# bartelvdh/Navtex

Measured on AMD Instinct MI355X. Metric: IQ Msamples/s through FIR->FSK->bitsync, higher is better.
Workload: dtype f64

## Files before the change

### navtex_amd/csrc/nvx_demod.hip

```cpp
#include <hip/hip_runtime.h>
#include <stdint.h>
#include <stdlib.h>

#include "nvx_tables.h"
#include "nvx_atan2.h"
#include "nvx_fsm.h"
#include "nvx_kernels.h"

enum { DS_Y3 = 0, DS_DPHI = 8, DS_S = 16, DS_C = 24, DS_COUNT = 24 + 567 };
enum { DI_SYNCED = 0, DI_SYNC_OFF, DI_NEXT_SYNC_OFF, DI_PHASE, DI_PREV_OFFSET, DI_COUNT };
static_assert(DI_COUNT == NVX_DEMOD_INTS && DS_COUNT == NVX_DEMOD_DOUBLES && DI_PREV_OFFSET == NVX_DI_PREV_OFFSET &&
              DI_PHASE == NVX_DI_PHASE, "state layout");

#ifndef NVX_FRONT_THREADS
#define NVX_FRONT_THREADS 128
#endif
#ifndef DTL
#define DTL NVX_FRONT_TILE
static_assert(DTL % 9 == 0, "a tile is a whole number of bit periods");
#endif
#define FRONT_SLIDE ((567 + NVX_FRONT_THREADS - 1) / NVX_FRONT_THREADS)
#define G_DAB 8
#define G_CB 574
#define G_CSA 582

__device__ __forceinline__ double2 y3_at(const double2 *y3, const double *hist, int t)
{
    if (t >= 0) return y3[t];
    double2 r; r.x = hist[2 * (4 + t)]; r.y = hist[2 * (4 + t) + 1];
    return r;
}

__device__ __forceinline__ double front_dphi(double2 s, double2 p)
{
    const double prodReal = s.x * p.x + s.y * p.y;
    const double prodImg  = s.y * p.x - s.x * p.y;
    return nvx_atan2(prodImg, prodReal);
}
__device__ __forceinline__ void front_energies(double2 w0, double2 w1, double2 w2, double2 w3, double2 w4,
                                               float &Brot, float &Yrot)
{
    float BR = 0.0f, BI = 0.0f, YR = 0.0f, YI = 0.0f;
#pragma unroll
    for (int i = 0; i < 5; i++) {
        const double2 w = i == 0 ? w0 : i == 1 ? w1 : i == 2 ? w2 : i == 3 ? w3 : w4;
        const float fR = NVX_BF_R[i], fI = NVX_BF_I[i];
        const double sampleR = w.x, sampleI = w.y;
        YR = (float)((double)YR + ((double)((float)sampleR * fR) - sampleI * (double)fI));
        YI = (float)((double)YI + ((double)((float)sampleR * fI) + sampleI * (double)fR));
        BR = (float)((double)BR + ((double)((float)sampleR * fR) + sampleI * (double)fI));
        BI = (float)((double)BI + ((double)((float)(-sampleR) * fI) + sampleI * (double)fR));
    }
    Brot = BR * BR + BI * BI;
    Yrot = YR * YR + YI * YI;
}
__device__ __forceinline__ unsigned char front_decision(double2 w0, double2 w1, double2 w2, double2 w3, double2 w4, float &hi, float &lo)
{
    float Brot, Yrot;
    front_energies(w0, w1, w2, w3, w4, Brot, Yrot);
    const bool b = Brot > Yrot;
    hi = b ? Brot : Yrot; lo = b ? Yrot : Brot;
    return b ? 1 : 0;
}

struct FrontSig { double power, dphi_b, dphi2_b, dphi_y, dphi2_y, hi, lo; unsigned nb, pad; };
__device__ __forceinline__ void front_sig_init(FrontSig &s)
{
    s.power = s.dphi_b = s.dphi2_b = s.dphi_y = s.dphi2_y = s.hi = s.lo = 0.0; s.nb = s.pad = 0;
}
__device__ __forceinline__ void front_sig_add(FrontSig &s, double2 y, double ds, unsigned char d, float hi, float lo)
{
    s.power += y.x * y.x + y.y * y.y;
    const double b = d ? ds : 0.0, m = d ? 0.0 : ds;
    s.dphi_b += b; s.dphi2_b += b * b; s.dphi_y += m; s.dphi2_y += m * m;
    s.hi += (double)hi; s.lo += (double)lo; s.nb += d;
}
__device__ __forceinline__ double front_wave_sum(double v)
{
#pragma unroll
    for (int o = 32; o >= 1; o >>= 1) v += __shfl_xor(v, o);
    return v;
}
__device__ __forceinline__ unsigned front_wave_sum(unsigned v)
{
#pragma unroll
    for (int o = 32; o >= 1; o >>= 1) v += __shfl_xor(v, o);
    return v;
}
__device__ __forceinline__ void front_sig_publish(FrontSig s, unsigned n, FrontSig *s_w, nvx_sig_rec *rec, int tid)
{
    s.power = front_wave_sum(s.power); s.dphi_b = front_wave_sum(s.dphi_b); s.dphi2_b = front_wave_sum(s.dphi2_b);
    s.dphi_y = front_wave_sum(s.dphi_y); s.dphi2_y = front_wave_sum(s.dphi2_y); s.hi = front_wave_sum(s.hi); s.lo = front_wave_sum(s.lo);
    s.nb = front_wave_sum(s.nb);
    if ((tid & 63) == 0) s_w[tid >> 6] = s;
    __syncthreads();
    if (tid == 0) {
        FrontSig t = s_w[0];
#pragma unroll
        for (int w = 1; w < NVX_FRONT_THREADS / 64; w++) {
            const FrontSig &u = s_w[w];
            t.power += u.power; t.dphi_b += u.dphi_b; t.dphi2_b += u.dphi2_b; t.dphi_y += u.dphi_y; t.dphi2_y += u.dphi2_y;
            t.hi += u.hi; t.lo += u.lo; t.nb += u.nb;
        }
        nvx_sig_rec r;
        r.sum_power = t.power; r.sum_dphi_b = t.dphi_b; r.sum_dphi2_b = t.dphi2_b; r.sum_dphi_y = t.dphi_y; r.sum_dphi2_y = t.dphi2_y;
        r.sum_mf_hi = t.hi; r.sum_mf_lo = t.lo; r.samples = n; r.b_samples = t.nb;
        *rec = r;
    }
}
__device__ __forceinline__ double front_corr(const double *dp)
{
    double temp = 0.0;
#pragma unroll
    for (int i = 0; i < 9; i++) temp += (double)NVX_CORR_MASK[i] * dp[i];
    return __builtin_fabs(temp);
}
__device__ __forceinline__ double front_class_sum(const double *cnow, unsigned u)
{
    const unsigned c = u % 9u;
    const int d0 = (int)((u + 566u - c) % 567u);
    const int jw = d0 / 9;
    const double *run1 = cnow - d0;
    const double *run2 = run1 - 567;
    double temp = 0.0;
#pragma unroll
    for (int j = 0; j < 63; j++) temp += (j <= jw ? run1 : run2)[9 * j];
    return temp;
}
struct FrontTies { unsigned near, evals; float minm; };
__device__ __forceinline__ FrontTies front_ties_init() { FrontTies t; t.near = 0; t.evals = 0; t.minm = __uint_as_float(0x7f800000u); return t; }
__device__ __forceinline__ unsigned short front_word(const unsigned char *d9, const double *sv, bool evaluate, FrontTies &ties)
{
    unsigned w = 0;
#pragma unroll
    for (int k = 0; k < 9; k++) w |= (unsigned)d9[k] << k;
    unsigned max_index = 15;
    if (evaluate) {
        double temp_max = -1.0, runner_up = -1.0;
        max_index = 0;
#pragma unroll
        for (int i = 0; i < 9; i++) {
            const double v = sv[i];
            if (v > temp_max) { runner_up = temp_max; temp_max = v; max_index = i; }
            else if (v > runner_up) runner_up = v;
        }
        if (temp_max > 0.0) {
            const double margin = temp_max - runner_up;
            ties.evals++;
            if (margin < temp_max * 0x1p-40) ties.near++;
            ties.minm = fminf(ties.minm, (float)(margin / temp_max));
        }
    }
    return (unsigned short)(w | (max_index << 12));
}

struct FrontChain { int slot; unsigned long long g0; const double *st_rd; double *st_wr; int n3; };
__device__ __forceinline__ FrontChain front_chain(const nvx_demod_args &a, int chain_index)
{
    FrontChain c;
    c.slot = chain_index; c.g0 = a.g0; c.n3 = a.n3;
    int parity = 0;
    if (a.part) {
        const int per = 2 * a.per_part, e = chain_index / per;
        c.slot = a.part[e].stream * per + (chain_index - e * per);
        c.g0 = a.part[e].g0; parity = a.part[e].parity; c.n3 = a.part[e].n3;
    }
    c.st_rd = (parity ? a.dstate[1] : a.dstate[0]) + (size_t)c.slot * NVX_DEMOD_DOUBLES;
    c.st_wr = (parity ? a.dstate[0] : a.dstate[1]) + (size_t)c.slot * NVX_DEMOD_DOUBLES;
    return c;
}

__device__ __forceinline__ void front_publish_ties(const nvx_demod_args &a, const FrontTies &t, unsigned *s_near, unsigned *s_evals, unsigned *s_minm, int tid)
{
    if (t.evals) { atomicAdd(s_near, t.near); atomicAdd(s_evals, t.evals); atomicMin(s_minm, __float_as_uint(t.minm)); }
    __syncthreads();
    if (tid == 0 && *s_evals) {
        if (*s_near) atomicAdd(&a.ties->near_ties, (unsigned long long)*s_near);
        atomicAdd(&a.ties->evaluations, (unsigned long long)*s_evals);
        atomicMin(&a.ties->min_margin_bits, *s_minm);
    }
}

struct FrontWalkLds {
    double dphi[8 + DTL];
    double S[8 + DTL];
    double C[567 + DTL];
    unsigned char D[DTL];
    unsigned near, evals, minm;
    FrontSig sig[NVX_FRONT_THREADS / 64];
};
template <bool SIG>
__device__ __forceinline__ void front_sequential(const nvx_demod_args &a, int chain_index, int n_tiles_here, FrontWalkLds &lds)
{
    double *const s_dphi = lds.dphi, *const s_S = lds.S, *const s_C = lds.C;
    unsigned char *const s_D = lds.D;
    unsigned &s_near = lds.near, &s_evals = lds.evals, &s_minm = lds.minm;
    const int tid = threadIdx.x;
    const FrontChain ch = front_chain(a, chain_index);
    const int slot = ch.slot;
    if (!a.slot_active[slot]) return;
    if (tid == 0) { s_near = 0; s_evals = 0; s_minm = 0x7f800000u; }
    FrontTies ties = front_ties_init();
    constexpr bool sig_on = SIG;
    FrontSig sig;
    front_sig_init(sig);

    const double *st = ch.st_rd;
    const double2 *y3 = a.y3 + (size_t)slot * a.y3_cap + a.y3_base;
    double *dphi_out = a.dphi ? a.dphi + (size_t)slot * a.y3_cap + a.y3_base : nullptr;
    double *corr_out = a.corr ? a.corr + (size_t)slot * a.y3_cap + a.y3_base : nullptr;
    double *csum_out = a.csum ? a.csum + (size_t)slot * a.y3_cap + a.y3_base : nullptr;
    const double *hist = st + DS_Y3;
    if (tid < 8) { s_dphi[tid] = st[DS_DPHI + tid]; s_S[tid] = st[DS_S + tid]; }
    for (int i = tid; i < 567; i += NVX_FRONT_THREADS) s_C[i] = st[DS_C + i];
    __syncthreads();

    const int n3 = ch.n3;
    const int n_here = n_tiles_here > 0 ? min(n3, n_tiles_here * DTL) : n3;
    for (int ta = 0; ta < n_here; ta += DTL) {
        const int tl = min(DTL, n_here - ta);
        const int tl9 = (tl + 8) / 9;
        const unsigned long long gt = ch.g0 + (unsigned long long)ta;
        for (int L = tid; L < tl; L += NVX_FRONT_THREADS) {
            const int t = ta + L;
            const double2 w3 = y3_at(y3, hist, t - 1), w4 = y3[t];
            const double ds = front_dphi(w4, w3);
            s_dphi[8 + L] = ds;
            if (dphi_out) dphi_out[t] = ds;
            float hi, lo;
            const unsigned char d = front_decision(y3_at(y3, hist, t - 4), y3_at(y3, hist, t - 3), y3_at(y3, hist, t - 2), w3, w4, hi, lo);
            s_D[L] = d;
            if (sig_on && gt + L >= G_DAB) front_sig_add(sig, w4, ds, d, hi, lo);
        }
        if (tid < 9 * tl9 - tl) s_D[tl + tid] = 0;
        __syncthreads();
        for (int L = tid; L < tl; L += NVX_FRONT_THREADS)
            s_C[567 + L] = (gt + L >= G_DAB) ? front_corr(&s_dphi[L]) : 0.0;
        __syncthreads();
        const unsigned t_cb = (unsigned)((gt % 5103u + (5103u - G_CB % 5103u)) % 5103u);
        for (int L = tid; L < tl; L += NVX_FRONT_THREADS)
            s_S[8 + L] = (gt + L >= G_CB) ? front_class_sum(&s_C[567 + L], t_cb + (unsigned)L) : 0.0;
        __syncthreads();
        if (corr_out)
            for (int L = tid; L < tl; L += NVX_FRONT_THREADS) { corr_out[ta + L] = s_C[567 + L]; csum_out[ta + L] = s_S[8 + L]; }
        for (int M = tid; M < tl9; M += NVX_FRONT_THREADS) {
            const int L = 9 * M + (G_CSA % 9);
            a.words[(size_t)slot * (a.y3_cap / 9) + (ta / 9 + M)] = front_word(&s_D[9 * M], &s_S[L], L < tl && gt + L >= G_CSA, ties);
        }
        __syncthreads();
        double h_d = 0.0, h_s = 0.0, h_c[FRONT_SLIDE];
        if (tid < 8) { h_d = s_dphi[tl + tid]; h_s = s_S[tl + tid]; }
#pragma unroll
        for (int k = 0; k < FRONT_SLIDE; k++) { const int i = tid + NVX_FRONT_THREADS * k; h_c[k] = (i < 567) ? s_C[tl + i] : 0.0; }
        __syncthreads();
        if (tid < 8) { s_dphi[tid] = h_d; s_S[tid] = h_s; }
#pragma unroll
        for (int k = 0; k < FRONT_SLIDE; k++) { const int i = tid + NVX_FRONT_THREADS * k; if (i < 567) s_C[i] = h_c[k]; }
        __syncthreads();
    }

    front_publish_ties(a, ties, &s_near, &s_evals, &s_minm, tid);
    if (sig_on) {
        const unsigned skip = ch.g0 >= G_DAB ? 0u : (unsigned)min((unsigned long long)n_here, G_DAB - ch.g0);
        front_sig_publish(sig, (unsigned)n_here - skip, lds.sig, a.sig_part + (size_t)slot * a.sig_stride, tid);
    }
    if (n_tiles_here > 0) return;
    double *sw = ch.st_wr;
    if (tid < 4 && n3 >= 4) { const double2 l = y3[n3 - 4 + tid]; sw[DS_Y3 + 2 * tid] = l.x; sw[DS_Y3 + 2 * tid + 1] = l.y; }
    if (tid < 8) { sw[DS_DPHI + tid] = s_dphi[tid]; sw[DS_S + tid] = s_S[tid]; }
    for (int i = tid; i < 567; i += NVX_FRONT_THREADS) sw[DS_C + i] = s_C[i];
}

__global__ __launch_bounds__(NVX_FRONT_THREADS) __attribute__((amdgpu_waves_per_eu(5))) void nvx_demod_front(nvx_demod_args a)
{
    __shared__ FrontWalkLds lds;
    if (a.sig) front_sequential<true>(a, blockIdx.x, 0, lds);
    else front_sequential<false>(a, blockIdx.x, 0, lds);
}

#define FRONT_LOOKBACK 576
__global__ __launch_bounds__(NVX_FRONT_THREADS) void nvx_demod_front_head(nvx_demod_args a)
{
    __shared__ FrontWalkLds lds;
    if (a.sig) front_sequential<true>(a, blockIdx.x, 2, lds);
    else front_sequential<false>(a, blockIdx.x, 2, lds);
}
__global__ __launch_bounds__(NVX_FRONT_THREADS) void nvx_demod_front_tiles(nvx_demod_args a, int wgs_per_chain)
{
    const int chain_index = blockIdx.x / wgs_per_chain, wg = blockIdx.x - chain_index * wgs_per_chain;
    __shared__ double p_dphi[FRONT_LOOKBACK + DTL];
    __shared__ double p_C[FRONT_LOOKBACK - 8 + DTL];
    __shared__ double p_S[2 + DTL];
    __shared__ unsigned char p_D[DTL];
    __shared__ unsigned s_near, s_evals, s_minm;
    __shared__ FrontSig s_sig[NVX_FRONT_THREADS / 64];
    const int tid = threadIdx.x;
    const FrontChain ch = front_chain(a, chain_index);
    const int slot = ch.slot;
    if (!a.slot_active[slot]) return;
    if (tid == 0) { s_near = 0; s_evals = 0; s_minm = 0x7f800000u; }
    FrontTies ties = front_ties_init();
    const int ta = (wg + 2) * DTL;
    const int tl = min(DTL, a.n3 - ta);
    const double2 *y3 = a.y3 + (size_t)slot * a.y3_cap + a.y3_base;
    double *dphi_out = a.dphi ? a.dphi + (size_t)slot * a.y3_cap + a.y3_base : nullptr;
    double *corr_out = a.corr ? a.corr + (size_t)slot * a.y3_cap + a.y3_base : nullptr;
    double *csum_out = a.csum ? a.csum + (size_t)slot * a.y3_cap + a.y3_base : nullptr;
    const unsigned long long g_ta = ch.g0 + (unsigned long long)ta;
    const bool sig_on = a.sig != nullptr;
    FrontSig sig;
    front_sig_init(sig);

    for (int i = tid; i < FRONT_LOOKBACK + tl; i += NVX_FRONT_THREADS) {
        const int t = ta - FRONT_LOOKBACK + i;
        const double ds = front_dphi(y3[t], y3[t - 1]);
        p_dphi[i] = ds;
        if (i >= FRONT_LOOKBACK) {
            if (dphi_out) dphi_out[t] = ds;
            float hi, lo;
            const unsigned char d = front_decision(y3[t - 4], y3[t - 3], y3[t - 2], y3[t - 1], y3[t], hi, lo);
            p_D[i - FRONT_LOOKBACK] = d;
            if (sig_on) front_sig_add(sig, y3[t], ds, d, hi, lo);
        }
    }
    __syncthreads();
    for (int i = tid; i < FRONT_LOOKBACK - 8 + tl; i += NVX_FRONT_THREADS)
        p_C[i] = (g_ta - 568 + (unsigned long long)i >= G_DAB) ? front_corr(&p_dphi[i]) : 0.0;
    __syncthreads();
    const unsigned t_cb = (unsigned)(((g_ta - 2) % 5103u + (5103u - G_CB % 5103u)) % 5103u);
    for (int i = tid; i < 2 + tl; i += NVX_FRONT_THREADS)
        p_S[i] = (g_ta - 2 + (unsigned long long)i >= G_CB) ? front_class_sum(&p_C[566 + i], t_cb + (unsigned)i) : 0.0;
    __syncthreads();
    if (corr_out)
        for (int i = tid; i < tl; i += NVX_FRONT_THREADS) { corr_out[ta + i] = p_C[FRONT_LOOKBACK - 8 + i]; csum_out[ta + i] = p_S[2 + i]; }
    for (int M = tid; M < tl / 9; M += NVX_FRONT_THREADS)
        a.words[(size_t)slot * (a.y3_cap / 9) + (ta / 9 + M)] = front_word(&p_D[9 * M], &p_S[9 * M], g_ta + 9 * M + (G_CSA % 9) >= G_CSA, ties);
    front_publish_ties(a, ties, &s_near, &s_evals, &s_minm, tid);
    if (sig_on) front_sig_publish(sig, (unsigned)tl, s_sig, a.sig_part + (size_t)slot * a.sig_stride + 1 + wg, tid);
    if (ta + tl >= a.n3) {
        double *sw = ch.st_wr;
        if (tid < 4) { const double2 l = y3[a.n3 - 4 + tid]; sw[DS_Y3 + 2 * tid] = l.x; sw[DS_Y3 + 2 * tid + 1] = l.y; }
        if (tid < 8) { sw[DS_DPHI + tid] = p_dphi[FRONT_LOOKBACK + tl - 8 + tid]; sw[DS_S + tid] = p_S[2 + tl - 8 + tid]; }
        for (int i = tid; i < 567; i += NVX_FRONT_THREADS) sw[DS_C + i] = p_C[FRONT_LOOKBACK - 8 + tl - 567 + i];
    }
}

#ifndef NVX_SOFT_INFLIGHT
#define NVX_SOFT_INFLIGHT 2
#endif
template <bool HIST>
__device__ __forceinline__ float fsm_soft_at(const double2 *y3, const double *hist, int t)
{
    double2 w[5];
#pragma unroll
    for (int i = 0; i < 5; i++) w[i] = HIST ? y3_at(y3, hist, t - 4 + i) : y3[t - 4 + i];
    float Brot, Yrot;
    front_energies(w[0], w[1], w[2], w[3], w[4], Brot, Yrot);
    return Brot - Yrot;
}
__device__ __forceinline__ int fsm_soft_period(const double2 *y3, const double *hist, int m, unsigned p, float *row, int cap, int j)
{
    const int n = NVX_FSM_POS_N(p);
    if (n >= 1) { const float v = fsm_soft_at<true>(y3, hist, 9 * m + NVX_FSM_POS_K1(p)); if (j < cap) row[j] = v; j++; }
    if (n == 2) { const float v = fsm_soft_at<true>(y3, hist, 9 * m + NVX_FSM_POS_K2(p)); if (j < cap) row[j] = v; j++; }
    return j;
}

template <bool SOFT>
__device__ __forceinline__ void fsm_chain(const nvx_demod_args &a, const uint32_t *s_tab)
{
    int slot = blockIdx.x * 64 + threadIdx.x;
    const int nc = a.n_slots;
    int n3 = a.n3, parity = 0;
    if (a.part) {
        const int per = 2 * a.per_part, e = slot / per;
        if (e >= a.n_part) return;
        slot = a.part[e].stream * per + (slot - e * per);
        n3 = a.part[e].n3; parity = a.part[e].parity;
    }
    if (slot >= nc) return;
    if (!a.slot_active[slot]) return;
    int *si = a.state_i;
#define SI(f) si[(size_t)(f) * nc + slot]
    nvx_fsm_regs r;
    r.so = SI(DI_SYNCED) ? SI(DI_SYNC_OFF) : NVX_FSM_UNSYNCED;
    r.nso = SI(DI_NEXT_SYNC_OFF);
    r.phase1 = SI(DI_PHASE) + 1;
    r.prev_offset = SI(DI_PREV_OFFSET);

    unsigned *bits = (unsigned *)(a.bits + (size_t)slot * a.bits_cap);
    const int cap_words = a.bits_cap / 4;
    unsigned long long acc = 0;
    int nacc = 0, nwords = 0;
    const int periods = n3 / 9;
    const unsigned short *wrow = a.words + (size_t)slot * (a.y3_cap / 9);
    const uint4 *words = (const uint4 *)wrow;
    uint4 wnext = words[0];
    unsigned short *prow = SOFT ? a.soft_pos + (size_t)slot * (a.y3_cap / 9) : nullptr;

    int m0 = 0;
    for (; m0 + 8 <= periods; m0 += 8) {
        const uint4 wv = wnext;
        if (m0 + 16 <= periods) wnext = words[m0 / 8 + 1];
        const unsigned wcur[8] = { wv.x & 0xffffu, wv.x >> 16, wv.y & 0xffffu, wv.y >> 16,
                                   wv.z & 0xffffu, wv.z >> 16, wv.w & 0xffffu, wv.w >> 16 };
        unsigned pcur[8];
#pragma unroll
        for (int i = 0; i < 8; i++) {
            int n;
            const unsigned b = nvx_fsm_period_pos(s_tab, wcur[i], &r, &n, &pcur[i]);
            acc |= (unsigned long long)(b & ((1u << n) - 1u)) << nacc;
            nacc += n;
        }
        if (SOFT) {
            uint4 pv;
            pv.x = pcur[0] | pcur[1] << 16; pv.y = pcur[2] | pcur[3] << 16; pv.z = pcur[4] | pcur[5] << 16; pv.w = pcur[6] | pcur[7] << 16;
            ((uint4 *)prow)[m0 / 8] = pv;
        }
        if (nacc >= 32) {
            if (nwords < cap_words) bits[nwords] = (unsigned)acc;
            nwords++; acc >>= 32; nacc -= 32;
        }
    }
    for (; m0 < periods; m0++) {
        int n;
        unsigned pos;
        const unsigned b = nvx_fsm_period_pos(s_tab, wrow[m0], &r, &n, &pos);
        if (SOFT) prow[m0] = (unsigned short)pos;
        acc |= (unsigned long long)(b & ((1u << n) - 1u)) << nacc;
        nacc += n;
        if (nacc >= 32) { if (nwords < cap_words) bits[nwords] = (unsigned)acc; nwords++; acc >>= 32; nacc -= 32; }
    }
    const int rem = n3 - 9 * periods;
    if (rem) {
        const unsigned w = wrow[periods];
        int n;
        unsigned pos;
        const unsigned b = nvx_fsm_partial_period_pos(w, rem, &r, &n, &pos);
        if (SOFT) prow[periods] = (unsigned short)pos;
        acc |= (unsigned long long)(b & ((1u << n) - 1u)) << nacc;
        nacc += n;
        if (nacc >= 32) { if (nwords < cap_words) bits[nwords] = (unsigned)acc; nwords++; acc >>= 32; nacc -= 32; }
    }
    if (nacc > 0 && nwords < cap_words) bits[nwords] = (unsigned)acc;

    a.nbits[slot] = nwords * 32 + nacc;
    const int synced = r.so != NVX_FSM_UNSYNCED;
    SI(DI_SYNCED) = synced; SI(DI_SYNC_OFF) = synced ? r.so : 0; SI(DI_NEXT_SYNC_OFF) = r.nso;
    SI(DI_PHASE) = r.phase1 - 1; SI(DI_PREV_OFFSET) = r.prev_offset;
#undef SI
    if (SOFT) {
        const double2 *y3 = a.y3 + (size_t)slot * a.y3_cap + a.y3_base;
        const double *hist = (parity ? a.dstate[1] : a.dstate[0]) + (size_t)slot * NVX_DEMOD_DOUBLES + DS_Y3;
        float *row = a.soft + (size_t)slot * a.soft_cap;
        const int cap = a.soft_cap;
        const int whole = periods & ~7;
        int j = 0, m = 0;
        const uint4 *notes = (const uint4 *)prow;
        if (whole) {
            const uint4 pv = notes[0];
            const unsigned pcur[8] = { pv.x & 0xffffu, pv.x >> 16, pv.y & 0xffffu, pv.y >> 16,
                                       pv.z & 0xffffu, pv.z >> 16, pv.w & 0xffffu, pv.w >> 16 };
#pragma unroll
            for (int i = 0; i < 8; i++) j = fsm_soft_period(y3, hist, i, pcur[i], row, cap, j);
            m = 8;
        }
        uint4 pnext = whole > 8 ? notes[1] : uint4{ 0, 0, 0, 0 };
        for (; m < whole; m += 8) {
            const uint4 pv = pnext;
            if (m + 16 <= whole) pnext = notes[m / 8 + 1];
            const unsigned pcur[8] = { pv.x & 0xffffu, pv.x >> 16, pv.y & 0xffffu, pv.y >> 16,
                                       pv.z & 0xffffu, pv.z >> 16, pv.w & 0xffffu, pv.w >> 16 };
#pragma unroll
            for (int i = 0; i < 8; i += NVX_SOFT_INFLIGHT) {
                float v[NVX_SOFT_INFLIGHT];
#pragma unroll
                for (int u = 0; u < NVX_SOFT_INFLIGHT; u++)
                    v[u] = fsm_soft_at<false>(y3, hist, 9 * (m + i + u) + (NVX_FSM_POS_N(pcur[i + u]) ? NVX_FSM_POS_K1(pcur[i + u]) : 8));
#pragma unroll
                for (int u = 0; u < NVX_SOFT_INFLIGHT; u++) {
                    const int n = NVX_FSM_POS_N(pcur[i + u]);
                    if (n >= 1) { if (j < cap) row[j] = v[u]; j++; }
                    if (n == 2) {
                        const float v2 = fsm_soft_at<false>(y3, hist, 9 * (m + i + u) + NVX_FSM_POS_K2(pcur[i + u]));
                        if (j < cap) row[j] = v2;
                        j++;
                    }
                }
            }
        }
        for (; m < periods + (rem ? 1 : 0); m++) j = fsm_soft_period(y3, hist, m, prow[m], row, cap, j);
    }
    if (a.sig) {
        const nvx_sig_rec *p = a.sig_part + (size_t)slot * a.sig_stride;
        nvx_sig_rec s = p[0];
        for (int k = 1; k < a.sig_parts; k++) {
            const nvx_sig_rec &q = p[k];
            s.sum_power += q.sum_power; s.sum_dphi_b += q.sum_dphi_b; s.sum_dphi2_b += q.sum_dphi2_b;
            s.sum_dphi_y += q.sum_dphi_y; s.sum_dphi2_y += q.sum_dphi2_y; s.sum_mf_hi += q.sum_mf_hi; s.sum_mf_lo += q.sum_mf_lo;
            s.samples += q.samples; s.b_samples += q.b_samples;
        }
        a.sig[slot] = s;
    }
}

__global__ __launch_bounds__(64) void nvx_demod_fsm(nvx_demod_args a)
{
    __shared__ uint32_t s_tab[NVX_FSM_TABLE_ALLOC];
    {
        const uint4 *src = (const uint4 *)a.fsm_table;
        uint4 *dst = (uint4 *)s_tab;
        for (int i = threadIdx.x; i < NVX_FSM_TABLE_ALLOC / 4; i += 64) dst[i] = src[i];
    }
    __syncthreads();
    if (a.soft) fsm_chain<true>(a, s_tab);
    else fsm_chain<false>(a, s_tab);
}

extern "C" int nvx_front_tile_wgs(const nvx_demod_args *a, int request)
{
    const unsigned chains = a->part ? (unsigned)(2 * a->per_part * a->n_part) : (unsigned)a->n_slots;
    const int tiles = (a->n3 + DTL - 1) / DTL;
    const long long chain_frames = (long long)chains * (a->n3 / NVX_Y3_PER_FRAME);
    const bool parallel = tiles >= 3 && (request >= 0 ? request != 0 : chain_frames <= 2560);
    return parallel ? tiles - 2 : 0;
}

extern "C" hipError_t nvx_launch_demod_front(const nvx_demod_args *a, hipStream_t s)
{
    const unsigned chains = a->part ? (unsigned)(2 * a->per_part * a->n_part) : (unsigned)a->n_slots;
    const int wgs = a->sig_parts - 1;
    if (wgs < 0) return hipErrorInvalidValue;
    if (a->sig && 1 + wgs > a->sig_stride) return hipErrorInvalidValue;
    if (wgs) {
        hipLaunchKernelGGL(nvx_demod_front_head, dim3(chains), dim3(NVX_FRONT_THREADS), 0, s, *a);
        hipLaunchKernelGGL(nvx_demod_front_tiles, dim3(chains * (unsigned)wgs), dim3(NVX_FRONT_THREADS), 0, s, *a, wgs);
    } else {
        hipLaunchKernelGGL(nvx_demod_front, dim3(chains), dim3(NVX_FRONT_THREADS), 0, s, *a);
    }
    return hipGetLastError();
}

extern "C" hipError_t nvx_launch_demod_fsm(const nvx_demod_args *a, hipStream_t s)
{
    const int chains = a->part ? 2 * a->per_part * a->n_part : a->n_slots;
    if (a->sig_parts < 1) return hipErrorInvalidValue;
    hipLaunchKernelGGL(nvx_demod_fsm, dim3((unsigned)((chains + 63) / 64)), dim3(64), 0, s, *a);
    return hipGetLastError();
}

extern "C" __attribute__((visibility("default"))) double nvx_atan2_host(double y, double x) { return nvx_atan2(y, x); }
```

Measured before the change: 1.535 million.

## Compute class sums with per-residue running prefixes plus a wave-level tail correction

Replaces the per-sample 63-term strided class sum with a running prefix along each of the nine residue classes. Nine threads carry these prefixes across tiles in LDS, borrowing the signature scratch area. Each wave then adds the remaining terms from the previous window in a bounded tail loop, with a uniform fast path where all lanes need the same count. Two block barriers in the tile-sliding step are dropped to cut synchronisation. The prefix chains are serial and run on only nine threads, which can leave the block idle on long tiles. Running sums also change the floating-point summation order.

Measured after the change: 1.541 million, median of 6. Within noise of the previous version (+0.4%).

```diff
diff --git a/navtex_amd/csrc/nvx_demod.hip b/navtex_amd/csrc/nvx_demod.hip
--- a/navtex_amd/csrc/nvx_demod.hip
+++ b/navtex_amd/csrc/nvx_demod.hip
@@ -127,6 +127,59 @@
     for (int j = 0; j < 63; j++) temp += (j <= jw ? run1 : run2)[9 * j];
     return temp;
 }
+__device__ __forceinline__ int front_class_jw(unsigned u) { return (int)((u / 9u + 62u) % 63u); }
+__device__ __forceinline__ double front_prefix_start(const double *s_C, unsigned t_cb, int r)
+{
+    const int jw = front_class_jw(t_cb + (unsigned)r);
+    const double *run1 = &s_C[567 + r - 8 - 9 * jw];
+    double temp = 0.0;
+    for (int j = 0; j < jw; j++) temp += run1[9 * j];
+    return temp;
+}
+#define FRONT_BATCH 8
+__device__ __forceinline__ double front_prefix_chain(double *s_S, const double *s_C, unsigned t_cb, int r, int tl, double p)
+{
+    int jw = front_class_jw(t_cb + (unsigned)r);
+    for (int L = r; L < tl; L += 9 * FRONT_BATCH) {
+        double x[FRONT_BATCH];
+#pragma unroll
+        for (int i = 0; i < FRONT_BATCH; i++) x[i] = s_C[567 - 8 + min(L + 9 * i, DTL - 1)];
+#pragma unroll
+        for (int i = 0; i < FRONT_BATCH; i++) {
+            p = (jw == 0 ? 0.0 : p) + x[i];
+            if (L + 9 * i < tl) s_S[8 + L + 9 * i] = p;
+            jw = jw == 62 ? 0 : jw + 1;
+        }
+    }
+    return p;
+}
+__device__ __forceinline__ void front_class_tail(double *s_S, const double *s_C, unsigned t_cb, int Lw, int lane, int tl, bool prim)
+{
+    const int Ll = min(Lw + 63, tl - 1);
+    const int jf = front_class_jw(t_cb + (unsigned)Lw), jl = front_class_jw(t_cb + (unsigned)Ll);
+    const int n_all = jl < jf ? 0 : 62 - jl, n_any = jl < jf ? 62 : 62 - jf;
+    const bool act = Lw + lane < tl;
+    const int L = act ? Lw + lane : Ll;
+    const int n = act ? 62 - front_class_jw(t_cb + (unsigned)L) : 0;
+    const double *c = &s_C[L + 1];
+    double s = s_S[8 + L];
+    int k = 0;
+    for (; k + FRONT_BATCH <= n_all; k += FRONT_BATCH) {
+        double x[FRONT_BATCH];
+#pragma unroll
+        for (int i = 0; i < FRONT_BATCH; i++) x[i] = c[9 * (k + i)];
+#pragma unroll
+        for (int i = 0; i < FRONT_BATCH; i++) s += x[i];
+    }
+    for (; k < n_any; k += FRONT_BATCH) {
+        double x[FRONT_BATCH];
+#pragma unroll
+        for (int i = 0; i < FRONT_BATCH; i++) x[i] = c[9 * min(k + i, 61)];
+#pragma unroll
+        for (int i = 0; i < FRONT_BATCH; i++) s += k + i < n ? x[i] : 0.0;
+    }
+    if (act) s_S[8 + L] = prim ? s : 0.0;
+}
 struct FrontTies { unsigned near, evals; float minm; };
 __device__ __forceinline__ FrontTies front_ties_init() { FrontTies t; t.near = 0; t.evals = 0; t.minm = __uint_as_float(0x7f800000u); return t; }
 __device__ __forceinline__ unsigned short front_word(const unsigned char *d9, const double *sv, bool evaluate, FrontTies &ties)
@@ -180,6 +233,8 @@
         atomicMin(&a.ties->min_margin_bits, *s_minm);
     }
 }
+
+__device__ __forceinline__ unsigned front_t_cb(unsigned long long gt) { return (unsigned)((gt % 5103u + (5103u - G_CB % 5103u)) % 5103u); }
 
 struct FrontWalkLds {
     double dphi[8 + DTL];
@@ -217,6 +272,9 @@
 
     const int n3 = ch.n3;
     const int n_here = n_tiles_here > 0 ? min(n3, n_tiles_here * DTL) : n3;
+    double *const s_pfx = reinterpret_cast<double *>(lds.sig);
+    static_assert(sizeof(lds.sig) >= 9 * sizeof(double), "room for nine prefixes");
+    if (tid < 9) s_pfx[tid] = front_prefix_start(s_C, front_t_cb(ch.g0), tid);
     for (int ta = 0; ta < n_here; ta += DTL) {
         const int tl = min(DTL, n_here - ta);
         const int tl9 = (tl + 8) / 9;
@@ -237,9 +295,14 @@
         for (int L = tid; L < tl; L += NVX_FRONT_THREADS)
             s_C[567 + L] = (gt + L >= G_DAB) ? front_corr(&s_dphi[L]) : 0.0;
         __syncthreads();
-        const unsigned t_cb = (unsigned)((gt % 5103u + (5103u - G_CB % 5103u)) % 5103u);
-        for (int L = tid; L < tl; L += NVX_FRONT_THREADS)
-            s_S[8 + L] = (gt + L >= G_CB) ? front_class_sum(&s_C[567 + L], t_cb + (unsigned)L) : 0.0;
+        const unsigned t_cb = front_t_cb(gt);
+        int tq = tid;
+        asm volatile("" : "+v"(tq));
+        if (tq < 9) s_pfx[tq] = front_prefix_chain(s_S, s_C, t_cb, tq, tl, s_pfx[tq]);
+        __syncthreads();
+        const int lane = tq & 63;
+        for (int Lw = __builtin_amdgcn_readfirstlane(tq - lane); Lw < tl; Lw += NVX_FRONT_THREADS)
+            front_class_tail(s_S, s_C, t_cb, Lw, lane, tl, gt + Lw + lane >= G_CB);
         __syncthreads();
         if (corr_out)
             for (int L = tid; L < tl; L += NVX_FRONT_THREADS) { corr_out[ta + L] = s_C[567 + L]; csum_out[ta + L] = s_S[8 + L]; }
@@ -247,7 +310,6 @@
             const int L = 9 * M + (G_CSA % 9);
             a.words[(size_t)slot * (a.y3_cap / 9) + (ta / 9 + M)] = front_word(&s_D[9 * M], &s_S[L], L < tl && gt + L >= G_CSA, ties);
         }
-        __syncthreads();
         double h_d = 0.0, h_s = 0.0, h_c[FRONT_SLIDE];
         if (tid < 8) { h_d = s_dphi[tl + tid]; h_s = s_S[tl + tid]; }
 #pragma unroll
@@ -256,7 +318,6 @@
         if (tid < 8) { s_dphi[tid] = h_d; s_S[tid] = h_s; }
 #pragma unroll
         for (int k = 0; k < FRONT_SLIDE; k++) { const int i = tid + NVX_FRONT_THREADS * k; if (i < 567) s_C[i] = h_c[k]; }
-        __syncthreads();
     }
 
     front_publish_ties(a, ties, &s_near, &s_evals, &s_minm, tid);
```
